# Chriz122/ultralytics_pro

Hardware: AMD Instinct MI355X
Metric: images/sec (whole job = n_gpus x per-GPU bs=32) YOLOv8n 640x640 (forward + Detect decode + NMS) (higher is better)
Workload: dtype bf16

## Files before the change

include/upa.h:

```cpp
#ifndef UPA_H
#define UPA_H
#include <stddef.h>
#include <stdint.h>

#ifdef __cplusplus
extern "C" {
#endif

enum { UPA_F32 = 0, UPA_BF16 = 1, UPA_U8_BGR_HWC = 2  };
enum { UPA_ACT_NONE = 0, UPA_ACT_SILU = 1, UPA_ACT_RELU = 2 };
enum { UPA_OK = 0, UPA_EINVAL = -1, UPA_EUNSUPPORTED = -2, UPA_EWORKSPACE = -3, UPA_ELAUNCH = -4 };

typedef struct upa_opts {
  uint32_t size;
  int32_t conv_big;
  int32_t conv_big_bm;
  int32_t conv_force[4];
  int32_t conv_ckt;
  int32_t no_ws, no_pipe, no_1x1, no_c16, no_upcat;
  int32_t pipe_all;
  int32_t pipe_min_tiles;
  int32_t pipe_wgs, c16_wgs;
  int32_t c1_mt, c1_waves, c1_wgs;
  int32_t pair;
  int32_t pair_tile64, pair_tile32;
  int32_t no_pair_cv2;
  int32_t c2f;
  int32_t c2f16_waves;
  int32_t c2f32_th;
  int32_t no_branch_tail;
  int32_t branch_tail_bm;
  int32_t stem_wgs, stemf_wgs, stemf_waves, stem_no_mfma;
  int32_t ablate_conv, ablate_pipe, ablate_c1, ablate_stem;
  int32_t c2f64_max_px;
  int32_t conv_ws3;
  int32_t no_group;
  int32_t no_c2f32_up;
  int32_t conv_mm;
  int32_t no_xcd;
  int32_t keys_only;
  int32_t conv_p8;
  int32_t c2f_stream;
  int32_t c2f_stream_rows;
  int32_t no_stack_first;
  int32_t no_epi_stats;
  int32_t nms_stages;
  int32_t nms_first_prefix;
  int32_t detect_stream;
  int32_t detect_stream_rows;
  int32_t no_sppf_front;
  int32_t no_c2f16_down;
} upa_opts;

int upa_version(void);
const char* upa_last_error(void);
size_t upa_opts_size(void);

size_t upa_conv_packed_weight_bytes(int cout, int cin, int k, int dtype);
int upa_pack_conv_weight(const float* w_oihw, int cout, int cin, int k, int dtype, void* out);
int upa_conv2d_bias_act(const void* x, int n, int h, int w, int cin, int ldx,
                        const void* w_packed, const float* bias ,
                        void* y, int cout, int ldy,
                        const void* residual , int ldr,
                        int k, int stride, int pad, int act, int dtype, const upa_opts* opts, void* stream);
typedef struct upa_conv_problem {
  const void* x; int32_t n, h, w, cin, ldx;
  const void* w_packed; const float* bias;
  void* y; int32_t cout, ldy;
  const void* residual; int32_t ldr;
} upa_conv_problem;
int upa_conv2d_bias_act_group(const upa_conv_problem* probs, int count, int k, int stride, int pad, int act, int dtype,
                              const upa_opts* opts, void* stream);

int upa_conv2d_pool2(const void* x, int n, int h, int w, int cin, int ldx, const void* w_packed, const float* bias, void* y, int cout,
                     int ldy, int k, int stride, int pad, int act, int dtype, const upa_opts* opts, void* stream);
int upa_conv2d_stem_nchw_pool2(const void* x_nchw, int x_dtype, int n, int cin, int h, int w, const float* w_oihw, const float* bias,
                               void* y, int cout, int ldy, int k, int stride, int pad, int act, int dtype, const upa_opts* opts,
                               void* stream);

int upa_conv_variant(int n, int h, int w, int cin, int cout, int k, int stride, int pad, int dtype, const upa_opts* opts);

int upa_bottleneck_pair(const void* x, int n, int h, int w, int c, int ldx, const void* w1_packed, const float* b1,
                        const void* w2_packed, const float* b2, void* y, int ldy, int residual, int act, int dtype,
                        const upa_opts* opts, void* stream);
// ... 19 lines not shown

int upa_maxpool2d(const void* x, int n, int h, int w, int c, int ldx, void* y, int oh, int ow, int ldy,
                  int k, int stride, int pad, int pad_br, int dtype, void* stream);
int upa_sppf_pool3(const void* x, int n, int h, int w, int c, int ldx, void* y1, void* y2, void* y3, int ldy,
                   int dtype, void* stream);
int upa_sppf_front(const void* x, int n, int h, int w, int c1, int ldx, const void* w_packed, const float* bias, void* y, int c_, int ldy, int dtype,
                   const upa_opts* opts, void* stream);
int upa_upsample2x(const void* x, int n, int h, int w, int c, int ldx, void* y, int ldy, int dtype, void* stream);
int upa_copy_view(const void* x, int n, int h, int w, int c, int ldx, void* y, int ldy, int dtype, void* stream);
int upa_copy_to_host(const void* src_dev, void* dst_pinned, size_t bytes, void* stream);
int upa_results_to_host(const void* rows_dev, const int* counts_dev, int batch, int max_rows, int row_bytes,
                        void* rows_pinned, int* counts_pinned, void* stream);
int upa_add_view(const void* a, int lda, const void* b, int ldb, void* y, int ldy, int n, int h, int w, int c,
                 int dtype, void* stream);
int upa_nchw_to_nhwc(const float* x, int n, int c, int h, int w, void* y, int ldy, int dtype, void* stream);
int upa_nhwc_to_nchw(const void* x, int n, int h, int w, int c, int ldx, float* y, int dtype, void* stream);
int upa_letterbox_u8(const void* src, int n, int h0, int w0, long src_image_stride, int src_row_stride, void* dst, int H, int W,
                     int new_h, int new_w, int top, int left, int pad_value, void* stream);


int upa_detect_decode(const void* box, int ldb, const void* cls, int ldc, int n, int h, int w, int reg_max, int nc,
                      float stride_px, float* y, int a_total, int a0, int dtype, void* stream);
int upa_detect_tail(const void* x, int n, int h, int w, int cin, int ldx, const void* w_packed, const float* bias, int cout,
                    int kind, int nc, float stride_px, float* y, int a_total, int a0, void* raw, int ldraw,
                    unsigned long long* best_keys, int dtype, const upa_opts* opts, void* stream);

int upa_conv1x1_upcat(const void* x, int n, int h, int w, int cin, int ldx, const void* up, int up_c, int up_ld,
                      const void* w_packed, const float* bias, void* y, int cout, int ldy, int act, int dtype,
                      const upa_opts* opts, void* stream);

int upa_bottleneck_pair_cv2(const void* x, const void* y0, int n, int h, int w, int ldx, const void* w1_packed, const float* b1,
                            const void* w2_packed, const float* b2, int residual, const void* wc_std, const void* wc_b,
                            const float* bc, void* out, int ldout, int act, int dtype, const upa_opts* opts, void* stream);

int upa_c2f_fused(const void* x, int n, int h, int w, int c1, int ldx, int c, int nb, int shortcut, const void* w1,
                  const float* b1, const void* const* wm, const float* const* bm, const void* w2, const float* b2, void* y,
                  int c2, int ldy, int act, int dtype, const upa_opts* opts, void* stream);

int upa_c2f16_down_fused(const void* x, int n, int h, int w, int ldx, const void* w1, const float* b1, const void* const* wm,
                         const float* const* bm, const void* w2, const float* b2, const void* wd, const float* bd, void* y, int ldy,
                         int dtype, const upa_opts* opts, void* stream);

int upa_c2f64_fused(const void* x, int n, int h, int w, int c1, int ldx, const void* up, int up_c, int up_ld, int nb, int shortcut,
                    const void* w1, const float* b1, const void* const* wm, const float* const* bm, const void* w2,
                    const float* b2, void* y, int c2, int ldy, int act, int dtype, const upa_opts* opts, void* stream);
int upa_c2f32_up_fused(const void* x, int n, int h, int w, int c1, int ldx, const void* up, int up_c, int up_ld, int nb, int shortcut,
                       const void* w1, const float* b1, const void* const* wm, const float* const* bm, const void* w2, const float* b2,
                       void* y, int c2, int ldy, int act, int dtype, const upa_opts* opts, void* stream);

size_t upa_tail_packed_weight_bytes(int cout, int cin);
int upa_pack_tail_weight(const float* w, int cout, int cin, void* out);
int upa_detect_branch_tail(const void* x, int n, int h, int w, int c, int ldx, const void* w3_packed, const float* b3,
                           const void* wt_packed, const float* bt, int kind, int nc, float stride_px, float* y, int a_total,
                           int a0, unsigned long long* best_keys, int dtype, const upa_opts* opts, void* stream);
typedef struct upa_branch_level {
  const void* x; int32_t n, h, w, c, ldx;
  const void* w3_packed; const float* b3;
  const void* wt_packed; const float* bt;
  float stride_px; int32_t a0;
} upa_branch_level;
int upa_detect_branch_tail_group(const upa_branch_level* levels, int count, int kind, int nc, float* y, int a_total,
                                 unsigned long long* best_keys, int dtype, const upa_opts* opts, void* stream);
int upa_detect_head_tails(const upa_branch_level* box, const upa_branch_level* cls, int count, int nc, float* y, int a_total,
                          unsigned long long* best_keys, int dtype, const upa_opts* opts, void* stream);
typedef struct upa_detect_branch {
  int32_t c, reserved;
// ... 139 lines not shown
```

ultralytics_pro_amd/_lib.py:

```python

from __future__ import annotations

import ctypes as C
import os
from pathlib import Path

import torch

UPA_F32, UPA_BF16, UPA_U8_BGR_HWC = 0, 1, 2
UPA_EUNSUPPORTED = -2
ACT_NONE, ACT_SILU, ACT_RELU = 0, 1, 2

_PKG = Path(__file__).resolve().parent
LIB_PATH = Path(os.environ.get("UPA_HIP_LIB", _PKG / "libupa_hip.so"))

_vp, _i, _f, _sz = C.c_void_p, C.c_int, C.c_float, C.c_size_t


class Opts(C.Structure):

    _fields_ = [("size", C.c_uint32), ("conv_big", _i), ("conv_big_bm", _i), ("conv_force", _i * 4), ("conv_ckt", _i),
                ("no_ws", _i), ("no_pipe", _i), ("no_1x1", _i), ("no_c16", _i), ("no_upcat", _i),
                ("pipe_all", _i), ("pipe_min_tiles", _i), ("pipe_wgs", _i), ("c16_wgs", _i),
                ("c1_mt", _i), ("c1_waves", _i), ("c1_wgs", _i),
                ("pair", _i), ("pair_tile64", _i), ("pair_tile32", _i), ("no_pair_cv2", _i),
                ("c2f", _i), ("c2f16_waves", _i), ("c2f32_th", _i),
                ("no_branch_tail", _i), ("branch_tail_bm", _i),
                ("stem_wgs", _i), ("stemf_wgs", _i), ("stemf_waves", _i), ("stem_no_mfma", _i),
                ("ablate_conv", _i), ("ablate_pipe", _i), ("ablate_c1", _i), ("ablate_stem", _i), ("c2f64_max_px", _i), ("conv_ws3", _i), ("no_group", _i), ("no_c2f32_up", _i), ("conv_mm", _i), ("no_xcd", _i), ("keys_only", _i), ("conv_p8", _i), ("c2f_stream", _i), ("c2f_stream_rows", _i), ("no_stack_first", _i), ("no_epi_stats", _i), ("nms_stages", _i), ("nms_first_prefix", _i), ("detect_stream", _i), ("detect_stream_rows", _i), ("no_sppf_front", _i), ("no_c2f16_down", _i)]

    def __init__(self, **kw):
        super().__init__()
        self.size = C.sizeof(Opts)
        for k, v in kw.items():
            if k == "conv_force":
                for j, x in enumerate(v):
                    self.conv_force[j] = int(x)
            elif k in dict(self._fields_):
                setattr(self, k, int(v))
            else:
                raise AttributeError(f"upa_opts has no field '{k}'")

    def replace(self, **kw) -> "Opts":
        o = Opts()
        C.memmove(C.byref(o), C.byref(self), C.sizeof(Opts))
        for k, v in kw.items():
            if k == "conv_force":
                for j, x in enumerate(v):
                    o.conv_force[j] = int(x)
            else:
                setattr(o, k, int(v))
        return o

    _ENV = {"UPA_CONV_BIG": ("conv_big", lambda v: {0: 1, 1: 0, 2: 2}[int(v)]), "UPA_CONV_BIG_BM": ("conv_big_bm", int), "UPA_CONV_WS3": ("conv_ws3", int),
            "UPA_CONV_CKT": ("conv_ckt", int), "UPA_CONV_NO_WS": ("no_ws", lambda v: 1), "UPA_CONV_NO_PIPE": ("no_pipe", lambda v: 1),
            "UPA_CONV_NO_1X1": ("no_1x1", lambda v: 1), "UPA_CONV_NO_C16": ("no_c16", lambda v: 1), "UPA_NO_UPCAT": ("no_upcat", lambda v: 1),
            "UPA_PIPE_ALL": ("pipe_all", lambda v: 1), "UPA_PIPE_MIN_TILES": ("pipe_min_tiles", int), "UPA_PIPE_WGS": ("pipe_wgs", int),
            "UPA_C16_WGS": ("c16_wgs", int), "UPA_C1_MT": ("c1_mt", int), "UPA_C1_WAVES": ("c1_waves", int), "UPA_C1_WGS": ("c1_wgs", int),
            "UPA_NO_PAIR": ("pair", lambda v: {0: 2, 1: 1, 2: 0, 3: 3}[int(v)]), "UPA_PAIR_T64": ("pair_tile64", int),
            "UPA_PAIR_T32": ("pair_tile32", int), "UPA_NO_PAIR_CV2": ("no_pair_cv2", int), "UPA_NO_C2F": ("c2f", int),
            "UPA_C2F16_WAVES": ("c2f16_waves", int), "UPA_C2F32_TH": ("c2f32_th", int), "UPA_NO_BRANCH_TAIL": ("no_branch_tail", int),
            "UPA_BRANCH_TAIL_BM": ("branch_tail_bm", int), "UPA_STEM_WGS": ("stem_wgs", int), "UPA_STEMF_WGS": ("stemf_wgs", int),
# ... 41 lines not shown
    "upa_conv_variant": (_i, [_i, _i, _i, _i, _i, _i, _i, _i, _i, _op]),
    "upa_bottleneck_pair": (_i, [_vp, _i, _i, _i, _i, _i, _vp, _vp, _vp, _vp, _vp, _i, _i, _i, _i, _op, _vp]),
    "upa_bottleneck_pair_e": (_i, [_vp, _i, _i, _i, _i, _i, _i, _vp, _vp, _vp, _vp, _vp, _i, _i, _i, _i, _op, _vp]),
    "upa_stem_packed_weight_bytes": (_sz, [_i, _i, _i]),
    "upa_pack_stem_weight": (_i, [_vp, _i, _i, _i, _vp]),
    "upa_conv2d_stem_nchw": (_i, [_vp, _i, _i, _i, _i, _i, _vp, _vp, _vp, _i, _i, _i, _i, _i, _i, _i, _op, _vp]),
    "upa_conv2d_stem_nchw_pool2": (_i, [_vp, _i, _i, _i, _i, _i, _vp, _vp, _vp, _i, _i, _i, _i, _i, _i, _i, _op, _vp]),
    "upa_conv2d_pool2": (_i, [_vp, _i, _i, _i, _i, _i, _vp, _vp, _vp, _i, _i, _i, _i, _i, _i, _i, _op, _vp]),
    "upa_stem_conv_fused": (_i, [_vp, _i, _i, _i, _vp, _vp, _vp, _vp, _vp, _i, _op, _vp]),
    "upa_stem_conv_fused_k": (_i, [_vp, _i, _i, _i, _i, _vp, _vp, _vp, _vp, _vp, _i, _op, _vp]),
    "upa_stem_conv_fused_c": (_i, [_vp, _i, _i, _i, _i, _i, _vp, _vp, _vp, _vp, _vp, _i, _op, _vp]),
    "upa_stem_conv_fused_s": (_i, [_vp, _i, _i, _i, _i, _i, _i, _vp, _vp, _vp, _vp, _vp, _i, _op, _vp]),
    "upa_maxpool2d": (_i, [_vp, _i, _i, _i, _i, _i, _vp, _i, _i, _i, _i, _i, _i, _i, _i, _vp]),
    "upa_sppf_pool3": (_i, [_vp, _i, _i, _i, _i, _i, _vp, _vp, _vp, _i, _i, _vp]),
    "upa_upsample2x": (_i, [_vp, _i, _i, _i, _i, _i, _vp, _i, _i, _vp]),
    "upa_copy_view": (_i, [_vp, _i, _i, _i, _i, _i, _vp, _i, _i, _vp]),
    "upa_copy_to_host": (_i, [_vp, _vp, _sz, _vp]),
    "upa_results_to_host": (_i, [_vp, _vp, _i, _i, _i, _vp, _vp, _vp]),
    "upa_add_view": (_i, [_vp, _i, _vp, _i, _vp, _i, _i, _i, _i, _i, _i, _vp]),
    "upa_nchw_to_nhwc": (_i, [_vp, _i, _i, _i, _i, _vp, _i, _i, _vp]),
    "upa_nhwc_to_nchw": (_i, [_vp, _i, _i, _i, _i, _i, _vp, _i, _vp]),
    "upa_letterbox_u8": (_i, [_vp, _i, _i, _i, C.c_long, _i, _vp, _i, _i, _i, _i, _i, _i, _i, _vp]),
    "upa_detect_decode": (_i, [_vp, _i, _vp, _i, _i, _i, _i, _i, _i, _f, _vp, _i, _i, _i, _vp]),
    "upa_detect_branch_tail_group": (_i, [_vp, _i, _i, _i, _vp, _i, _vp, _i, _op, _vp]),
    "upa_detect_head_tails": (_i, [_vp, _vp, _i, _i, _vp, _i, _vp, _i, _op, _vp]),
    "upa_conv2d_bias_act_group": (_i, [_vp, _i, _i, _i, _i, _i, _i, _op, _vp]),
    "upa_detect_level_stream": (_i, [_vp, _i, _i, _i, _i, _i, _vp, _vp, _i, _f, _vp, _i, _i, _vp, _i, _op, _vp]),
    "upa_detect_tail": (_i, [_vp, _i, _i, _i, _i, _i, _vp, _vp, _i, _i, _i, _f, _vp, _i, _i, _vp, _i, _vp, _i, _op, _vp]),
    "upa_conv1x1_upcat": (_i, [_vp, _i, _i, _i, _i, _i, _vp, _i, _i, _vp, _vp, _vp, _i, _i, _i, _i, _op, _vp]),
    "upa_bottleneck_pair_cv2": (_i, [_vp, _vp, _i, _i, _i, _i, _vp, _vp, _vp, _vp, _i, _vp, _vp, _vp, _vp, _i, _i, _i, _op, _vp]),
    "upa_sppf_front": (_i, [_vp, _i, _i, _i, _i, _i, _vp, _vp, _vp, _i, _i, _i, _op, _vp]),
    "upa_c2f16_down_fused": (_i, [_vp, _i, _i, _i, _i, _vp, _vp, _vp, _vp, _vp, _vp, _vp, _vp, _vp, _i, _i, _op, _vp]),
    "upa_c2f_fused": (_i, [_vp, _i, _i, _i, _i, _i, _i, _i, _i, _vp, _vp, _vp, _vp, _vp, _vp, _vp, _i, _i, _i, _i, _op, _vp]),
    "upa_c2f64_fused": (_i, [_vp, _i, _i, _i, _i, _i, _vp, _i, _i, _i, _i, _vp, _vp, _vp, _vp, _vp, _vp, _vp, _i, _i, _i, _i, _op, _vp]),
    "upa_c2f32_up_fused": (_i, [_vp, _i, _i, _i, _i, _i, _vp, _i, _i, _i, _i, _vp, _vp, _vp, _vp, _vp, _vp, _vp, _i, _i, _i, _i, _op, _vp]),
    "upa_tail_packed_weight_bytes": (_sz, [_i, _i]),
    "upa_pack_tail_weight": (_i, [_vp, _i, _i, _vp]),
    "upa_detect_branch_tail": (_i, [_vp, _i, _i, _i, _i, _i, _vp, _vp, _vp, _vp, _i, _i, _f, _vp, _i, _i, _vp, _i, _op, _vp]),
    "upa_nms_batched_hot": (_i, [_vp, _i, _i, _i, _f, _f, _i, _i, _vp, _i, _i, _f, _vp, _vp, _vp, _vp, _sz, _vp, _vp]),
    "upa_nms_workspace_bytes": (_sz, [_i, _i, _i, _i, _i]),
    "upa_nms_batched": (_i, [_vp, _i, _i, _i, _f, _f, _i, _i, _vp, _i, _i, _f, _vp, _vp, _vp, _vp, _sz, _vp]),
    "upa_nms_batched_opts": (_i, [_vp, _i, _i, _i, _f, _f, _i, _i, _vp, _i, _i, _f, _vp, _vp, _vp, _vp, _sz, _vp, _vp]),
    "upa_mhsa": (_i, [_vp, _vp, _vp, _i, _i, _i, _i, _i, _f, _vp, _i, _vp, _i, _i, _vp]),
    "upa_linear": (_i, [_vp, C.c_long, _i, _i, _vp, _vp, _vp, _i, _i, _vp, _i, _i, _vp]),
    "upa_linear_bf16": (_i, [_vp, C.c_long, _i, _i, _vp, _vp, _vp, _i, _i, _vp, _i, _i, _vp]),
    "upa_linear_mixed": (_i, [_vp, _i, C.c_long, _i, _i, _vp, _vp, _vp, _i, _i, _i, _vp, _i, _i, _vp]),
    "upa_layer_norm": (_i, [_vp, _vp, _i, _i, _vp, _vp, _f, _vp, _vp]),
    "upa_rows_add": (_i, [_vp, _vp, _vp, C.c_long, _i, _vp]),
    "upa_rows_scale": (_i, [_vp, _vp, _vp, C.c_long, _i, _vp]),
    "upa_rows_gather": (_i, [_vp, _vp, _vp, C.c_long, _i, _vp]),
    "upa_topk_tokens": (_i, [_vp, _i, _i, _vp, _i, _i, _vp, _vp, _vp]),
    "upa_box_refine": (_i, [_vp, _vp, _vp, C.c_long, _vp]),
    "upa_box_add_anchors": (_i, [_vp, _vp, _vp, _vp, C.c_long, _vp]),
    "upa_sigmoid": (_i, [_vp, _vp, C.c_long, _vp]),
    "upa_rtdetr_output": (_i, [_vp, _vp, _vp, C.c_long, _i, _vp]),
    "upa_rtdetr_postprocess": (_i, [_vp, _i, _i, _i, _f, _vp, _i, _vp, _f, _f, _vp, _vp, _vp]),
    "upa_msdeform_attn": (_i, [_vp, _vp, _i, _i, _i, _i, _vp, _vp, _vp, _i, _i, _vp, _vp]),
    "upa_msdeform_attn_strided": (_i, [_vp, _i, _i, _vp, _i, _i, _i, _i, _vp, _vp, _vp, _i, _i, _vp, _vp]),
    "upa_box_iou": (_i, [_vp, _i, _vp, _i, _f, _vp, _vp]),
    "upa_match_predictions": (_i, [_vp, _vp, _i, _i, _vp, _vp, _i, _vp, _i, _vp, _vp]),
    "upa_scale_boxes": (_i, [_vp, C.c_long, _i, _f, _f, _f, _i, _f, _f, _vp]),
    "upa_pack_conv_weight_dev": (_i, [_vp, _i, _i, _i, _i, _i, _vp, _vp]),
    "upa_channel_reduce_workspace_bytes": (_sz, [_i]),
    "upa_bn_stats": (_i, [_vp, C.c_long, _i, _i, _vp, _i, _vp]),
    "upa_bn_finalize": (_i, [_vp, C.c_long, _i, _f, _vp, _vp, _vp, _vp, _vp]),
    "upa_conv2d_bn_act_fwd": (_i, [_vp, _i, _i, _i, _i, _i, _vp, _vp, _i, _i, _i, _i, _i, _f, _vp, _vp, _vp, _vp, _vp, _vp, _f, _i, _vp, _i, _vp, _i,
# ... 80 lines not shown
```

ultralytics_pro_amd/csrc/conv_big.hip:

```cpp
#include <stdlib.h>

#include <mutex>
#include <type_traits>
#include <unordered_map>

#include "common.h"
#include "conv_pipe.h"
UPA_STAMP_DEFINE(conv_big)

typedef __attribute__((address_space(1))) const void* bgptr_t;
typedef __attribute__((address_space(3))) void* blptr_t;

__device__ __attribute__((aligned(16))) unsigned g_big_zero16[4] = {0u, 0u, 0u, 0u};

namespace {
template <int ACT>
__device__ __forceinline__ float big_act(float v) {
  if constexpr (ACT == UPA_ACT_SILU) return v * __builtin_amdgcn_rcpf(1.0f + __expf(-v));
  else if constexpr (ACT == UPA_ACT_RELU) return fmaxf(v, 0.0f);
  else return v;
}
}

template <int KS, int STRIDE, int WM, int WN, int MT, int NT, int TAIL = 0>
__device__ __forceinline__ void conv_big_body(const BigParams& p, const int bid0) {
  static_assert(WM * WN == 8, "8 waves per workgroup");
  static_assert(TAIL == 0 || TAIL == 3 || TAIL == 4 || WN == 1, "a tail needs every channel of a pixel in one wave");
  static_assert(TAIL != 1 || (NT % 2) == 0, "box branch: 64 channels");
  static_assert(TAIL != 3 || (NT % 2) == 0, "the statistics epilogue pairs n-tiles");
  static_assert(TAIL != 4 || ((NT % 2) == 0 && KS == 2 && STRIDE == 1), "the interleaving epilogue: 2 x 2 phase kernels, paired n-tiles");
  constexpr int NTB = WN * NT;
  constexpr int WBUF = 2 * NTB * 1024;
  extern __shared__ __attribute__((aligned(16))) char smem[];
  const int tid = threadIdx.x;
  const int lane = tid & 63;
  const int wave = __builtin_amdgcn_readfirstlane(tid >> 6);
  const int r = lane & 15, g = lane >> 4;
  const int wm = wave / WN, wn = wave % WN;

  const int tilesPerImg = p.tilesX * p.tilesY;
  int bid = p.no_xcd ? bid0 : upa_xcd_tile(bid0, tilesPerImg * p.N);
  const int n = bid / tilesPerImg;
  bid -= n * tilesPerImg;
  const int tyi = bid / p.tilesX;
  const int txi = bid - tyi * p.tilesX;
  const int oy0 = tyi * p.TH, ox0 = txi * p.TW;
  const int iy0 = oy0 * STRIDE - p.pad, ix0 = ox0 * STRIDE - p.pad;
  const int ntb0 = blockIdx.y * NTB;

  const int haloItems = p.IH * p.IWp * 8;
  const int haloPadded = (haloItems + 63) & ~63;
  char* hal = smem;
  char* wbuf = smem + (size_t)haloPadded * 16;

  int pl0[MT], pty[MT], ptx[MT];
#pragma unroll
  for (int i = 0; i < MT; ++i) {
    const int pp = (wm * MT + i) * 16 + r;
    int ty = (int)__umulhi((unsigned)pp, p.magicTW);
    int tx = pp - ty * p.TW;
// ... 87 lines not shown
                                                                  *reinterpret_cast<const bf16x8*>(&b[i]), acc[i][j], 0, 0, 0);
        } else {
          constexpr int GS = (NT + 1) / 2;
          u32x4 b[MT];
#pragma unroll
          for (int i = 0; i < MT; ++i) b[i] = *reinterpret_cast<const u32x4*>(hal + paddr[i] + (((kt * 4 + g) ^ pswz[i]) << 4));
#pragma unroll
          for (int j0 = 0; j0 < NT; j0 += GS) {
            u32x4 a[GS];
#pragma unroll
            for (int j = 0; j < GS; ++j)
              if (j0 + j < NT) a[j] = *reinterpret_cast<const u32x4*>(wb + (kt * NTB + j0 + j) * 1024);
#pragma unroll
            for (int i = 0; i < MT; ++i)
#pragma unroll
              for (int j = 0; j < GS; ++j)
                if (j0 + j < NT)
                  acc[i][j0 + j] = __builtin_amdgcn_mfma_f32_16x16x32_bf16(*reinterpret_cast<const bf16x8*>(&a[j]),
                                                                           *reinterpret_cast<const bf16x8*>(&b[i]), acc[i][j0 + j], 0, 0, 0);
            __builtin_amdgcn_sched_barrier(0);
          }
        }
      }
      buf ^= 1;
      if (++kw == KS) { kw = 0; ++kh; }
    }
    if (c + 1 < nChunks) {
      __syncthreads();
      stage_halo(c + 1);
      stage_w(c + 1, 0, buf);
    }
  }
  UPA_STAMP_AT(10);

  if constexpr (TAIL == 1 || TAIL == 2) {
    f32x4 bv[NT];
#pragma unroll
    for (int j = 0; j < NT; ++j) bv[j] = *reinterpret_cast<const f32x4*>(p.bias + j * 16 + g * 4);
    f32x4 acc2[MT][NT];
#pragma unroll
    for (int i = 0; i < MT; ++i)
#pragma unroll
      for (int j = 0; j < NT; ++j) acc2[i][j] = f32x4{0.f, 0.f, 0.f, 0.f};
#pragma unroll
    for (int s2 = 0; s2 < NT / 2; ++s2) {
      u32x4 hb[MT];
#pragma unroll
      for (int i = 0; i < MT; ++i) {
        float v0[4], v1[4];
#pragma unroll
        for (int q = 0; q < 4; ++q) {
          v0[q] = big_act<UPA_ACT_SILU>(acc[i][2 * s2][q] + bv[2 * s2][q]);
          v1[q] = big_act<UPA_ACT_SILU>(acc[i][2 * s2 + 1][q] + bv[2 * s2 + 1][q]);
        }
        hb[i] = u32x4{pack_bf16x2(v0[0], v0[1]), pack_bf16x2(v0[2], v0[3]), pack_bf16x2(v1[0], v1[1]), pack_bf16x2(v1[2], v1[3])};
      }
#pragma unroll
      for (int j = 0; j < NT; ++j) {
        const u32x4 a2 = *reinterpret_cast<const u32x4*>(p.tw + ((size_t)(s2 * NT + j) * 64 + lane) * 16);
#pragma unroll
        for (int i = 0; i < MT; ++i)
          acc2[i][j] = __builtin_amdgcn_mfma_f32_16x16x32_bf16(*reinterpret_cast<const bf16x8*>(&a2),
                                                               *reinterpret_cast<const bf16x8*>(&hb[i]), acc2[i][j], 0, 0, 0);
      }
    }
    if constexpr (NT & 1) {
// ... 714 lines not shown
      memset(&o, 0, sizeof(o));
      if (opts) memcpy(&o, opts, opts->size < sizeof(o) ? opts->size : sizeof(o));
      o.size = sizeof(o);
      o.conv_big_bm = 128;
      p[0] = probs[0];
      rc = big_prepare(p[0], ntb[0], bm[0], lds[0], &o, false);
    }
    if (rc == UPA_OK && bm[0] == 128 && ntb[0] == ntb[1]) {
      const size_t l3 = lds[0] > lds[1] ? (lds[0] > lds[2] ? lds[0] : lds[2]) : (lds[1] > lds[2] ? lds[1] : lds[2]);
      rc = ntb[0] == 4 ? big_launch_tri_inst<3, 1, 4, 2, 2, 2>(p[0], p[1], p[2], l3, s) : big_launch_tri_inst<3, 1, 8, 1, 1, 5>(p[0], p[1], p[2], l3, s);
      if (rc == UPA_OK) { *consumed = 3; return UPA_OK; }
      if (rc != UPA_EUNSUPPORTED) return rc;
    }
    p[0] = probs[0];
    if (const int rc2 = big_prepare(p[0], ntb[0], bm[0], lds[0], opts, false); rc2 != UPA_OK) return rc2;
  }
  if (ok_ntb(ntb[0]) && ok_ntb(ntb[1]) && bm[0] == bm[1] && (bm[0] == 128 || bm[0] == 256)) {
    if (ntb[0] != ntb[1]) {
      const int lo = ntb[0] < ntb[1] ? 0 : 1;
      p[lo] = probs[lo];
      int bmf = 0;
      if (const int rc = big_prepare(p[lo], ntb[lo], bmf, lds[lo], opts, false, 5); rc != UPA_OK) return rc;
      if (bmf != bm[1 - lo] || ntb[lo] != 5) return UPA_EUNSUPPORTED;
    }
    const size_t l2 = lds[0] > lds[1] ? lds[0] : lds[1];
    int rc;
    if (bm[0] == 128) rc = ntb[0] == 4 ? big_launch_pair_inst<3, 1, 4, 2, 2, 2>(p[0], p[1], l2, s) : big_launch_pair_inst<3, 1, 8, 1, 1, 5>(p[0], p[1], l2, s);
    else rc = ntb[0] == 4 ? big_launch_pair_inst<3, 1, 8, 1, 2, 4>(p[0], p[1], l2, s) : big_launch_pair_inst<3, 1, 8, 1, 2, 5>(p[0], p[1], l2, s);
    if (rc == UPA_OK) { *consumed = 2; return UPA_OK; }
    if (rc != UPA_EUNSUPPORTED) return rc;
  }
  return UPA_EUNSUPPORTED;
}
```

ultralytics_pro_amd/csrc/conv_pipe.h:

```cpp
#pragma once
struct PipeParams {
  const char* x;
  char* y;
  const char* res;
  const char* w;
  const float* bias;
  int N, H, W, Cin, ldx, Cout, ldy, ldr;
  int KTT, NTn, nt0;
  int tilesX, tilesY, numTiles;
  int act;
  int pool;
#ifdef UPA_ABLATE
  int ablate;
#endif
};
bool upa_conv_pipe_eligible(int n, int h, int w, int cin, int ldx, int cout, int ldy, int ldr, int k, int stride, int pad,
                            int act, int dtype, const upa_opts* opts);
int upa_conv_pipe_launch(PipeParams p, int query_only, int* variant, void* stream, const upa_opts* opts);

#include "detect_epi.h"
struct C1Params {
  const char* x;
  char* y;
  const char* w;
// ... 9 lines not shown
  DetectEpi de;
  float* stats;
  int stats_ld;
  const char* up;
  int upKT, up_ld, upH, upW;
  unsigned upMagicW, upMagicH;
};
bool upa_conv1x1_eligible(int n, int h, int w, int cin, int ldx, int cout, int ldy, bool residual, int k, int stride,
                          int pad, int act, int dtype, const upa_opts* opts);
int upa_conv1x1_launch(C1Params p, int n_pixels, int query_only, int* variant, void* stream, const upa_opts* opts);
int upa_conv1x1_launch_stats(C1Params p, int n_pixels, int* rows, long max_rows, void* stream, const upa_opts* opts);

struct BigParams {
  const char* x;
  char* y;
  const char* res;
  const char* w;
  const float* bias;
  int N, H, W, Cin, ldx, OH, OW, Cout, ldy, ldr;
  int KS, stride, pad;
  int TH, TW, tilesX, tilesY, IH, IW;
  int IWp;
  int HALF;
  int KTT, NTn;
  int act;
  unsigned magicTW, magicIW;
  int no_xcd;
  const char* tw;
  const float* tb;
  DetectEpi de;
  float* stats;
  int stats_ld;
  int il_h, il_w, il_c;
};
bool upa_conv_big_eligible(int n, int h, int w, int cin, int ldx, int cout, int ldy, int ldr, int k, int stride, int pad,
                           int act, int dtype, const upa_opts* opts);
int upa_conv_big_launch(BigParams p, int query_only, int* variant, void* stream, const upa_opts* opts);
int upa_conv_big_launch_stats(BigParams p, int* rows, long max_rows, void* stream, const upa_opts* opts);
int upa_conv_big_launch_interleave(BigParams p, void* stream, const upa_opts* opts);
int upa_conv_big_launch_group(const BigParams* probs, int count, int* consumed, void* stream, const upa_opts* opts);

bool upa_conv_big_pick_tile(BigParams& p, int bm, int ntb, size_t lds_cap);

bool upa_conv_p8_eligible(int n, int h, int w, int cin, int ldx, int cout, int ldy, int ldr, int k, int stride, int pad, int act,
                          int dtype, const upa_opts* opts);
int upa_conv_p8_launch(BigParams p, int query_only, int* variant, void* stream, const upa_opts* opts);

bool upa_conv_mm_eligible(int n, int h, int w, int cin, int ldx, int cout, int ldy, int ldr, int k, int stride, int pad, int act,
                          int dtype, const upa_opts* opts);
int upa_conv_mm_launch(BigParams p, int query_only, int* variant, void* stream, const upa_opts* opts);

bool upa_conv_ws3_eligible(int n, int h, int w, int cin, int ldx, int cout, int ldy, bool residual, int k, int stride, int pad,
                           int act, int dtype, const upa_opts* opts);
int upa_conv_ws3_launch(BigParams p, int query_only, int* variant, void* stream, const upa_opts* opts);
int upa_conv_ws3_launch_stats(BigParams p, int* rows, long max_rows, void* stream, const upa_opts* opts);

struct PairParams {
  const char* x;
  char* y;
  const char* w1;
  const char* w2;
  const float* b1;
  const float* b2;
  int N, H, W, OH, OW, ldx, ldy;
  int TH, TW, tilesX, tilesY;
  int IWp, MWp;
// ... 8 lines not shown
```

ultralytics_pro_amd/nn/modules/block.py:

```python

from __future__ import annotations

import torch
import torch.nn as nn

from ... import _lib as L
from ...engine import runtime as R
from .conv import Conv, PackedConv, _HipConvMixin, fold_bn, hip_conv2d, version_key

__all__ = ("DFL", "SPPF", "C2f", "C3", "Bottleneck", "MHSA", "BottleneckTransformer", "BoT3")


class DFL(nn.Module):

    def __init__(self, c1: int = 16):
        super().__init__()
        self.conv = nn.Conv2d(c1, 1, 1, bias=False).requires_grad_(False)
        self.conv.weight.data[:] = torch.arange(c1, dtype=torch.float).view(1, c1, 1, 1)
        self.c1 = c1

    def forward(self, x):
        raise L.UpaError("DFL is fused into upa_detect_decode on the HIP path; call Detect instead")


# ... 120 lines not shown
        n, _, h, w = x.shape
        oh, ow = (h + 1) // 2, (w + 1) // 2
        y = out if out is not None else R.alloc_nhwc(n, 64, oh, ow, x.dtype, x.device, key=(id(down), "y"))
        pk = [cv._packed(cv.conv, cv.bn, x.device, x.dtype, False) for cv in convs]
        wm = (C.c_void_p * 2)(pk[2].w.data_ptr(), pk[3].w.data_ptr())
        bm = (C.c_void_p * 2)(pk[2].bias.data_ptr(), pk[3].bias.data_ptr())
        vx, vy = R.view_of(x), R.view_of(y)
        rc = L.lib().upa_c2f16_down_fused(vx.ptr, vx.n, vx.h, vx.w, vx.ld, pk[0].w.data_ptr(), pk[0].bias.data_ptr(), C.cast(wm, C.c_void_p),
                                          C.cast(bm, C.c_void_p), pk[1].w.data_ptr(), pk[1].bias.data_ptr(), pk[4].w.data_ptr(),
                                          pk[4].bias.data_ptr(), vy.ptr, vy.ld, vx.dtype, R.opts_ptr(), L.current_stream(x.device))
        if rc == 0:
            return y
        if rc != L.UPA_EUNSUPPORTED:
            L.check(rc, "c2f16_down_fused")
        return None

    def forward(self, x, out=None, up=None):
        x = R.to_nhwc(x, x.dtype)
        if up is not None and self.fuse_block and self.cv1.conv.in_channels in (32, 64) and not (self._form64() or self._form32up()):
            up.materialize()
            up = None
        y = self._fused(x, out, up)
        if y is not None:
            return y
        if up is not None and up.done:
            up = None
        n, _, h, w = x.shape
        c, nb = self.c, len(self.m)
        cat = R.alloc_nhwc(n, (2 + nb) * c, h, w, x.dtype, x.device, key=(id(self), "cat"))
        self.cv1(x, out=cat[:, : 2 * c], up=up)
        y = self._pair_cv2(cat, out)
        if y is not None:
            return y
        for i, m in enumerate(self.m):
            m(cat[:, (1 + i) * c: (2 + i) * c], out=cat[:, (2 + i) * c: (3 + i) * c])
        return self.cv2(cat, out=out)

    fuse_pair_cv2 = True

    def invalidate_packed(self):
        self.__dict__.pop("_pc_cache", None)

    def train(self, mode: bool = True):
        self.invalidate_packed()
        return super().train(mode)

    def _pair_cv2(self, cat, out):
        m = self.m[0] if len(self.m) == 1 else None
        if not (self.fuse_pair_cv2 and m is not None and self.c == 32 and self.cv2.conv.out_channels == 64
                and cat.dtype == torch.bfloat16 and not self.training and m._pair_ok(cat[:, 32:64])
                and isinstance(self.cv2.act, nn.SiLU) and self.cv2.conv.kernel_size == (1, 1) and hasattr(self.cv2, "bn")):
            return None
        n, _, h, w = cat.shape
        dev = cat.device
        y = out if out is not None else R.alloc_nhwc(n, 64, h, w, cat.dtype, dev, key=(id(self), "y"))
        p1 = m.cv1._packed(m.cv1.conv, m.cv1.bn, dev, cat.dtype, False)
        p2 = m.cv2._packed(m.cv2.conv, m.cv2.bn, dev, cat.dtype, False)
        cache = self.__dict__.setdefault("_pc_cache", {})
        cv = self.cv2
        ver = version_key(cv.conv.weight, cv.conv.bias, cv.bn.weight, cv.bn.bias, cv.bn.running_mean, cv.bn.running_var) + (cv.bn.eps,)
        hit = cache.get(str(dev))
        if hit is None or hit[0] != ver:
            wf, bf = fold_bn(cv.conv, cv.bn)
            std = PackedConv(wf[:, :64].contiguous(), bf, 1, dev, cat.dtype, False)
            wb = wf[:, 64:96].reshape(64, 32).contiguous().float()
            host = torch.empty(L.lib().upa_tail_packed_weight_bytes(64, 32), dtype=torch.uint8)
            L.check(L.lib().upa_pack_tail_weight(wb.data_ptr(), 64, 32, host.data_ptr()), "pack_tail_weight")
            hit = (ver, std, host.to(dev))
            cache[str(dev)] = hit
# ... 191 lines not shown
```

Before: 60720.

## Fuse last Bottleneck 3x3 conv with C2f cv2 1x1 projection in one kernel

Adds a TAIL==5 epilogue to the big conv kernel. It computes the last Bottleneck's 3x3 conv (with residual) for 128 pixels by 64 channels, keeps the result in LDS, and then runs the C2f cv2 1x1 conv over the earlier concat channels plus that on-chip result. This drops the global write and re-read of the last bottleneck output and one kernel launch per qualifying C2f. The path only applies to small bf16 maps with c=64 and c2=128, where the grid is smaller than the CU count. It costs extra LDS and a serial second GEMM inside each workgroup.

```diff
diff --git a/include/upa.h b/include/upa.h
--- a/include/upa.h
+++ b/include/upa.h
@@ -50,6 +50,7 @@
   int32_t detect_stream_rows;
   int32_t no_sppf_front;
   int32_t no_c2f16_down;
+  int32_t c2f_tails;
 } upa_opts;
 
 int upa_version(void);
@@ -135,6 +136,11 @@
 int upa_bottleneck_pair_cv2(const void* x, const void* y0, int n, int h, int w, int ldx, const void* w1_packed, const float* b1,
                             const void* w2_packed, const float* b2, int residual, const void* wc_std, const void* wc_b,
                             const float* bc, void* out, int ldout, int act, int dtype, const upa_opts* opts, void* stream);
+
+int upa_c2f_cv2_tail_form(int n, int h, int w, int c, int kc, int c2, int dtype, const upa_opts* opts);
+int upa_c2f_cv2_tail(const void* x, int n, int h, int w, int c, int ldx, const void* w3_packed, const float* b3, const void* residual,
+                     int ldr, const void* cat, int kc, int ldc, const void* w2_packed, const float* b2, void* y, int c2, int ldy, int act,
+                     int dtype, const upa_opts* opts, void* stream);
 
 int upa_c2f_fused(const void* x, int n, int h, int w, int c1, int ldx, int c, int nb, int shortcut, const void* w1,
                   const float* b1, const void* const* wm, const float* const* bm, const void* w2, const float* b2, void* y,
diff --git a/ultralytics_pro_amd/_lib.py b/ultralytics_pro_amd/_lib.py
--- a/ultralytics_pro_amd/_lib.py
+++ b/ultralytics_pro_amd/_lib.py
@@ -27,7 +27,7 @@
                 ("c2f", _i), ("c2f16_waves", _i), ("c2f32_th", _i),
                 ("no_branch_tail", _i), ("branch_tail_bm", _i),
                 ("stem_wgs", _i), ("stemf_wgs", _i), ("stemf_waves", _i), ("stem_no_mfma", _i),
-                ("ablate_conv", _i), ("ablate_pipe", _i), ("ablate_c1", _i), ("ablate_stem", _i), ("c2f64_max_px", _i), ("conv_ws3", _i), ("no_group", _i), ("no_c2f32_up", _i), ("conv_mm", _i), ("no_xcd", _i), ("keys_only", _i), ("conv_p8", _i), ("c2f_stream", _i), ("c2f_stream_rows", _i), ("no_stack_first", _i), ("no_epi_stats", _i), ("nms_stages", _i), ("nms_first_prefix", _i), ("detect_stream", _i), ("detect_stream_rows", _i), ("no_sppf_front", _i), ("no_c2f16_down", _i)]
+                ("ablate_conv", _i), ("ablate_pipe", _i), ("ablate_c1", _i), ("ablate_stem", _i), ("c2f64_max_px", _i), ("conv_ws3", _i), ("no_group", _i), ("no_c2f32_up", _i), ("conv_mm", _i), ("no_xcd", _i), ("keys_only", _i), ("conv_p8", _i), ("c2f_stream", _i), ("c2f_stream_rows", _i), ("no_stack_first", _i), ("no_epi_stats", _i), ("nms_stages", _i), ("nms_first_prefix", _i), ("detect_stream", _i), ("detect_stream_rows", _i), ("no_sppf_front", _i), ("no_c2f16_down", _i), ("c2f_tails", _i)]
 
     def __init__(self, **kw):
         super().__init__()
@@ -135,6 +135,8 @@
     "upa_sppf_front": (_i, [_vp, _i, _i, _i, _i, _i, _vp, _vp, _vp, _i, _i, _i, _op, _vp]),
     "upa_c2f16_down_fused": (_i, [_vp, _i, _i, _i, _i, _vp, _vp, _vp, _vp, _vp, _vp, _vp, _vp, _vp, _i, _i, _op, _vp]),
     "upa_c2f_fused": (_i, [_vp, _i, _i, _i, _i, _i, _i, _i, _i, _vp, _vp, _vp, _vp, _vp, _vp, _vp, _i, _i, _i, _i, _op, _vp]),
+    "upa_c2f_cv2_tail_form": (_i, [_i, _i, _i, _i, _i, _i, _i, _op]),
+    "upa_c2f_cv2_tail": (_i, [_vp, _i, _i, _i, _i, _i, _vp, _vp, _vp, _i, _vp, _i, _i, _vp, _vp, _vp, _i, _i, _i, _i, _op, _vp]),
     "upa_c2f64_fused": (_i, [_vp, _i, _i, _i, _i, _i, _vp, _i, _i, _i, _i, _vp, _vp, _vp, _vp, _vp, _vp, _vp, _i, _i, _i, _i, _op, _vp]),
     "upa_c2f32_up_fused": (_i, [_vp, _i, _i, _i, _i, _i, _vp, _i, _i, _i, _i, _vp, _vp, _vp, _vp, _vp, _vp, _vp, _i, _i, _i, _i, _op, _vp]),
     "upa_tail_packed_weight_bytes": (_sz, [_i, _i]),
diff --git a/ultralytics_pro_amd/csrc/conv_big.hip b/ultralytics_pro_amd/csrc/conv_big.hip
--- a/ultralytics_pro_amd/csrc/conv_big.hip
+++ b/ultralytics_pro_amd/csrc/conv_big.hip
@@ -25,7 +25,9 @@
 template <int KS, int STRIDE, int WM, int WN, int MT, int NT, int TAIL = 0>
 __device__ __forceinline__ void conv_big_body(const BigParams& p, const int bid0) {
   static_assert(WM * WN == 8, "8 waves per workgroup");
-  static_assert(TAIL == 0 || TAIL == 3 || TAIL == 4 || WN == 1, "a tail needs every channel of a pixel in one wave");
+  static_assert(TAIL == 0 || TAIL == 3 || TAIL == 4 || TAIL == 5 || WN == 1, "a tail needs every channel of a pixel in one wave");
+  static_assert(TAIL != 5 || (KS == 3 && STRIDE == 1 && WM == 4 && WN == 2 && MT == 2 && NT == 2),
+                "the C2f cv2 tail: 128 pixels x all 64 channels of the last Bottleneck per workgroup");
   static_assert(TAIL != 1 || (NT % 2) == 0, "box branch: 64 channels");
   static_assert(TAIL != 3 || (NT % 2) == 0, "the statistics epilogue pairs n-tiles");
   static_assert(TAIL != 4 || ((NT % 2) == 0 && KS == 2 && STRIDE == 1), "the interleaving epilogue: 2 x 2 phase kernels, paired n-tiles");
@@ -179,6 +181,138 @@
     }
   }
   UPA_STAMP_AT(10);
+
+  if constexpr (TAIL == 5) {
+    constexpr int NT2 = 4, NTB2 = 8, OBUF = 128 * 128, WBUF2 = 2 * NTB2 * 1024;
+    char* obuf = smem;
+    char* wbuf2 = smem + 2 * OBUF;
+    const int nmem = p.K2 >> 6;
+    const int nch2 = nmem + 1;
+    int pq[MT];
+#pragma unroll
+    for (int i = 0; i < MT; ++i) pq[i] = (wm * MT + i) * 16 + r;
+
+    auto stage_x2 = [&](int c, int b) __attribute__((always_inline)) {
+#pragma unroll
+      for (int k = 0; k < 2; ++k) {
+        const int base = k * 512 + wave * 64;
+        const int idx = base + lane;
+        const int q = idx >> 3;
+        const int cg = (idx & 7) ^ (q & 7);
+        const int ty = (int)__umulhi((unsigned)q, p.magicTW);
+        const int tx = q - ty * p.TW;
+        const int oy = oy0 + ty, ox = ox0 + tx;
+        const char* src = reinterpret_cast<const char*>(g_big_zero16);
+        if (ty < p.TH && oy < p.OH && ox < p.OW)
+          src = p.x2 + ((((size_t)n * p.OH + oy) * p.OW + ox) * (size_t)p.ldx2 + c * 64 + cg * 8) * 2;
+        __builtin_amdgcn_global_load_lds((bgptr_t)src, (blptr_t)(obuf + b * OBUF + base * 16), 16, 0, 0);
+      }
+    };
+    auto stage_w2 = [&](int c, int b) __attribute__((always_inline)) {
+#pragma unroll
+      for (int f0 = 0; f0 < 2 * NTB2; f0 += 8) {
+        const int f = f0 + wave;
+        const int kt = f / NTB2, j = f - kt * NTB2;
+        const char* src = p.tw + (((size_t)(c * 2 + kt) * NTB2 + j) * 64 + lane) * 16;
+        __builtin_amdgcn_global_load_lds((bgptr_t)src, (blptr_t)(wbuf2 + b * WBUF2 + f * 1024), 16, 0, 0);
+      }
+    };
+    auto store_b = [&](int b) __attribute__((always_inline)) {
+      const int cw = wn * NT * 16;
+      const f32x4 bj0 = *reinterpret_cast<const f32x4*>(p.bias + cw + g * 4), bj1 = *reinterpret_cast<const f32x4*>(p.bias + cw + 16 + g * 4);
+      const int cb = 16 * (g & 1) + 8 * (g >> 1);
+#pragma unroll
+      for (int i = 0; i < MT; ++i) {
+        const int oy = oy0 + pty[i], ox = ox0 + ptx[i];
+        const bool pok = pty[i] < p.TH && oy < p.OH && ox < p.OW;
+        float v0[4], v1[4], x8[8];
+#pragma unroll
+        for (int q = 0; q < 4; ++q) {
+          v0[q] = big_act<UPA_ACT_SILU>(acc[i][0][q] + bj0[q]);
+          v1[q] = big_act<UPA_ACT_SILU>(acc[i][1][q] + bj1[q]);
+        }
+#pragma unroll
+        for (int q = 0; q < 4; ++q) {
+          auto sw = __builtin_amdgcn_permlane16_swap(__float_as_uint(v0[q]), __float_as_uint(v1[q]), false, false);
+          x8[q] = __uint_as_float(sw[0]);
+          x8[4 + q] = __uint_as_float(sw[1]);
+        }
+        if (p.res && pok) {
+          const size_t pixoff = ((size_t)n * p.OH + oy) * p.OW + ox;
+          const u32x4 rv = *reinterpret_cast<const u32x4*>(p.res + (pixoff * p.ldr + cw + cb) * 2);
+#pragma unroll
+          for (int q = 0; q < 4; ++q) {
+            x8[2 * q] += __uint_as_float(rv[q] << 16);
+            x8[2 * q + 1] += __uint_as_float(rv[q] & 0xFFFF0000u);
+          }
+        }
+        *reinterpret_cast<u32x4*>(obuf + b * OBUF + pq[i] * 128 + ((((cw + cb) >> 3) ^ (pq[i] & 7)) << 4)) =
+            u32x4{pack_bf16x2(x8[0], x8[1]), pack_bf16x2(x8[2], x8[3]), pack_bf16x2(x8[4], x8[5]), pack_bf16x2(x8[6], x8[7])};
+      }
+    };
+
+    f32x4 acc2[MT][NT2];
+#pragma unroll
+    for (int i = 0; i < MT; ++i)
+#pragma unroll
+      for (int j = 0; j < NT2; ++j) acc2[i][j] = f32x4{0.f, 0.f, 0.f, 0.f};
+    __syncthreads();
+    stage_x2(0, 0);
+    stage_w2(0, 0);
+#pragma unroll 1
+    for (int c = 0; c < nch2; ++c) {
+      const int b = c & 1;
+      asm volatile("s_waitcnt vmcnt(0)" ::: "memory");
+      __syncthreads();
+      if (c + 1 < nch2) {
+        stage_w2(c + 1, b ^ 1);
+        if (c + 1 < nmem) stage_x2(c + 1, b ^ 1);
+        else store_b(b ^ 1);
+      }
+      const char* ob = obuf + b * OBUF;
+      const char* wb = wbuf2 + b * WBUF2 + (wn * NT2) * 1024 + lane * 16;
+#pragma unroll
+      for (int kt = 0; kt < 2; ++kt) {
+        u32x4 a[NT2], bb[MT];
+#pragma unroll
+        for (int j = 0; j < NT2; ++j) a[j] = *reinterpret_cast<const u32x4*>(wb + (kt * NTB2 + j) * 1024);
+#pragma unroll
+        for (int i = 0; i < MT; ++i) bb[i] = *reinterpret_cast<const u32x4*>(ob + pq[i] * 128 + (((kt * 4 + g) ^ (pq[i] & 7)) << 4));
+#pragma unroll
+        for (int i = 0; i < MT; ++i)
+#pragma unroll
+          for (int j = 0; j < NT2; ++j)
+            acc2[i][j] = __builtin_amdgcn_mfma_f32_16x16x32_bf16(*reinterpret_cast<const bf16x8*>(&a[j]),
+                                                                 *reinterpret_cast<const bf16x8*>(&bb[i]), acc2[i][j], 0, 0, 0);
+      }
+    }
+    const int cw2 = wn * NT2 * 16;
+    f32x4 tbv[NT2];
+#pragma unroll
+    for (int j = 0; j < NT2; ++j) tbv[j] = *reinterpret_cast<const f32x4*>(p.tb + cw2 + j * 16 + g * 4);
+#pragma unroll
+    for (int i = 0; i < MT; ++i) {
+      const int oy = oy0 + pty[i], ox = ox0 + ptx[i];
+      const bool pok = pty[i] < p.TH && oy < p.OH && ox < p.OW;
+      const size_t pixoff = ((size_t)n * p.OH + oy) * p.OW + ox;
+      char* yrow = p.y + (pixoff * p.ldy + cw2) * 2;
+#pragma unroll
+      for (int j = 0; j < NT2; j += 2) {
+        const int cb = 16 * (j + (g & 1)) + 8 * (g >> 1);
+        float v0[4], v1[4];
+#pragma unroll
+        for (int q = 0; q < 4; ++q) {
+          v0[q] = big_act<UPA_ACT_SILU>(acc2[i][j][q] + tbv[j][q]);
+          v1[q] = big_act<UPA_ACT_SILU>(acc2[i][j + 1][q] + tbv[j + 1][q]);
+        }
+        auto lo = __builtin_amdgcn_permlane16_swap(pack_bf16x2(v0[0], v0[1]), pack_bf16x2(v1[0], v1[1]), false, false);
+        auto hi = __builtin_amdgcn_permlane16_swap(pack_bf16x2(v0[2], v0[3]), pack_bf16x2(v1[2], v1[3]), false, false);
+        if (pok) *reinterpret_cast<u32x4*>(yrow + cb * 2) = u32x4{lo[0], hi[0], lo[1], hi[1]};
+      }
+    }
+    UPA_STAMP_AT(11);
+    return;
+  }
 
   if constexpr (TAIL == 1 || TAIL == 2) {
     f32x4 bv[NT];
@@ -959,3 +1093,47 @@
   }
   return UPA_EUNSUPPORTED;
 }
+
+namespace {
+bool c2f_tail_form(int n, int h, int w, int c, int kc, int c2, int dtype, const upa_opts* opts) {
+  if (UPA_OPT(opts, c2f_tails) == 1 || dtype != UPA_BF16 || c != 64 || c2 != 128 || kc < 64 || kc % 64 != 0 || kc > 1024) return false;
+  if (n <= 0 || h <= 0 || w <= 0) return false;
+  const long px = (long)n * h * w;
+  return px < (1L << 30) && (px + 255) / 256 < big_num_cu();
+}
+}
+
+extern "C" int upa_c2f_cv2_tail_form(int n, int h, int w, int c, int kc, int c2, int dtype, const upa_opts* opts) {
+  return c2f_tail_form(n, h, w, c, kc, c2, dtype, opts) ? 1 : 0;
+}
+
+extern "C" int upa_c2f_cv2_tail(const void* x, int n, int h, int w, int c, int ldx, const void* w3_packed, const float* b3,
+                                const void* residual, int ldr, const void* cat, int kc, int ldc, const void* w2_packed, const float* b2,
+                                void* y, int c2, int ldy, int act, int dtype, const upa_opts* opts, void* stream) {
+  UPA_CHECK_ARG(x && w3_packed && b3 && cat && w2_packed && b2 && y, "c2f_cv2_tail: null pointer");
+  if (!c2f_tail_form(n, h, w, c, kc, c2, dtype, opts) || act != UPA_ACT_SILU || ldx % 8 != 0 || ldc % 8 != 0 || ldy % 8 != 0 ||
+      ldx < c || ldc < kc || ldy < c2 || (residual && (ldr % 8 != 0 || ldr < c || (uintptr_t)residual % 16 != 0)) ||
+      (uintptr_t)x % 16 != 0 || (uintptr_t)cat % 16 != 0 || (uintptr_t)y % 16 != 0) {
+    upa_set_error("c2f_cv2_tail: outside the fused form (bf16 SiLU, c = 64, cv2 (kc + 64) -> 128, kc %% 64 == 0, 16-byte rows, "
+                  "small maps, upa_opts.c2f_tails != 1)");
+    return UPA_EUNSUPPORTED;
+  }
+  BigParams p;
+  memset(&p, 0, sizeof(p));
+  p.x = (const char*)x; p.y = (char*)y; p.res = (const char*)residual; p.w = (const char*)w3_packed; p.bias = b3;
+  p.N = n; p.H = h; p.W = w; p.Cin = c; p.ldx = ldx; p.OH = h; p.OW = w; p.Cout = c; p.ldy = ldy; p.ldr = ldr;
+  p.KS = 3; p.stride = 1; p.pad = 1; p.act = UPA_ACT_SILU;
+  p.KTT = cdiv(c, 32);
+  p.NTn = cdiv(c, 16);
+  p.tw = (const char*)w2_packed; p.tb = b2;
+  p.x2 = (const char*)cat; p.ldx2 = ldc; p.K2 = kc;
+  p.no_xcd = UPA_OPT(opts, no_xcd);
+  constexpr size_t tail_lds = 4 * 16384;
+  if (!big_pick_tile(p, 128, 4, 80 * 1024 - 512) && !big_pick_tile(p, 128, 4, 160 * 1024)) return UPA_EUNSUPPORTED;
+  p.tilesX = cdiv(p.OW, p.TW);
+  p.tilesY = cdiv(p.OH, p.TH);
+  size_t lds = big_halo_bytes(p) + 2 * (size_t)(2 * 4 * 1024);
+  lds = (lds > tail_lds ? lds : tail_lds) + 256;
+  if (lds > 160 * 1024) return UPA_EUNSUPPORTED;
+  return big_launch_inst<3, 1, 4, 2, 2, 2, 5>(p, lds, (hipStream_t)stream);
+}
diff --git a/ultralytics_pro_amd/csrc/conv_pipe.h b/ultralytics_pro_amd/csrc/conv_pipe.h
--- a/ultralytics_pro_amd/csrc/conv_pipe.h
+++ b/ultralytics_pro_amd/csrc/conv_pipe.h
@@ -65,6 +65,8 @@
   float* stats;
   int stats_ld;
   int il_h, il_w, il_c;
+  const char* x2;
+  int ldx2, K2;
 };
 bool upa_conv_big_eligible(int n, int h, int w, int cin, int ldx, int cout, int ldy, int ldr, int k, int stride, int pad,
                            int act, int dtype, const upa_opts* opts);
diff --git a/ultralytics_pro_amd/nn/modules/block.py b/ultralytics_pro_amd/nn/modules/block.py
--- a/ultralytics_pro_amd/nn/modules/block.py
+++ b/ultralytics_pro_amd/nn/modules/block.py
@@ -176,9 +176,46 @@
         y = self._pair_cv2(cat, out)
         if y is not None:
             return y
-        for i, m in enumerate(self.m):
+        for i, m in enumerate(self.m[:-1]):
             m(cat[:, (1 + i) * c: (2 + i) * c], out=cat[:, (2 + i) * c: (3 + i) * c])
+        y = self._cv2_tail(cat, out)
+        if y is not None:
+            return y
+        self.m[-1](cat[:, nb * c: (nb + 1) * c], out=cat[:, (nb + 1) * c:])
         return self.cv2(cat, out=out)
+
+    fuse_cv2_tail = True
+
+    def _cv2_tail(self, cat, out):
+        if not self.m:
+            return None
+        m, cv = self.m[-1], self.cv2
+        nb, c = len(self.m), self.c
+        n, _, h, w = cat.shape
+        if not (self.fuse_cv2_tail and cat.dtype == torch.bfloat16 and not self.training
+                and L.lib().upa_c2f_cv2_tail_form(n, h, w, c, (1 + nb) * c, cv.conv.out_channels, L.UPA_BF16, R.opts_ptr()) == 1
+                and all(isinstance(k.act, nn.SiLU) and hasattr(k, "bn") and k.conv.groups == 1 and k.conv.dilation == (1, 1)
+                        and k.conv.stride == (1, 1) for k in (m.cv1, m.cv2, cv))
+                and m.cv2.conv.kernel_size == (3, 3) and m.cv2.conv.padding == (1, 1) and m.cv2.conv.in_channels == c
+                and m.cv2.conv.out_channels == c and cv.conv.kernel_size == (1, 1) and cv.conv.in_channels == (2 + nb) * c):
+            return None
+        dev = cat.device
+        xin = cat[:, nb * c: (nb + 1) * c]
+        t = m.cv1(xin)
+        y = out if out is not None else R.alloc_nhwc(n, cv.conv.out_channels, h, w, cat.dtype, dev, key=(id(self), "y"))
+        p3 = m.cv2._packed(m.cv2.conv, m.cv2.bn, dev, cat.dtype, False)
+        p2 = cv._packed(cv.conv, cv.bn, dev, cat.dtype, False)
+        vt, vx, vc, vy = R.view_of(t), R.view_of(xin), R.view_of(cat), R.view_of(y)
+        rc = L.lib().upa_c2f_cv2_tail(vt.ptr, vt.n, vt.h, vt.w, vt.c, vt.ld, p3.w.data_ptr(), p3.bias.data_ptr(),
+                                      vx.ptr if m.add else None, vx.ld if m.add else 0, vc.ptr, (1 + nb) * c, vc.ld,
+                                      p2.w.data_ptr(), p2.bias.data_ptr(), vy.ptr, vy.c, vy.ld, L.ACT_SILU, vt.dtype, R.opts_ptr(),
+                                      L.current_stream(dev))
+        if rc == 0:
+            return y
+        if rc != L.UPA_EUNSUPPORTED:
+            L.check(rc, "c2f_cv2_tail")
+        m.cv2(t, out=cat[:, (nb + 1) * c:], residual=xin if m.add else None)
+        return cv(cat, out=out)
 
     fuse_pair_cv2 = True
 
```

Result: no change. 61300 (median of 6 runs) (+0.9%).
